# Benny44/QPALM

Measured on AMD Instinct MI355X. Metric: QP solves/sec (batched random n=1000,m=2000); `value` = solve only, batch resident in HBM -- with qpalm_setup in the clock as the reference's run_time has it: `value_setup_plus_solve`, higher is better.
Workload: dtype f64

## Files before the change

### qpalm_amd/csrc/qpalm_dense.h

```cpp
#ifndef QPALM_DENSE_H
#define QPALM_DENSE_H
#include <type_traits>

#ifdef QPALM_EMU
#define QP_FLAG_LOAD(p) (*(volatile int *)(p))
#define QP_FLAG_STORE(p, v) (*(volatile int *)(p) = (v))
#define QP_RELEASE_AGENT() do { } while (0)
#define QP_ACQUIRE_AGENT() do { } while (0)
#define QP_DRAIN_VMEM() do { } while (0)
#define QP_SLEEP() do { } while (0)
#define QP_WAVE_SYNC() emu_wave_sync()
#define QP_LDS_VBASE(p) (p)
#define QP_SCHED_BARRIER() do { } while (0)
#define QP_SETPRIO(p) do { } while (0)
#define QP_DRAIN_LDS() do { } while (0)
#else
#define QP_FLAG_LOAD(p) __hip_atomic_load((p), __ATOMIC_RELAXED, __HIP_MEMORY_SCOPE_AGENT)
#define QP_FLAG_STORE(p, v) __hip_atomic_store((p), (v), __ATOMIC_RELAXED, __HIP_MEMORY_SCOPE_AGENT)
#define QP_RELEASE_AGENT() __builtin_amdgcn_fence(__ATOMIC_RELEASE, "agent")
#define QP_ACQUIRE_AGENT() __builtin_amdgcn_fence(__ATOMIC_ACQUIRE, "agent")
#define QP_DRAIN_VMEM() asm volatile("s_waitcnt vmcnt(0)" ::: "memory")
#define QP_SLEEP() __builtin_amdgcn_s_sleep(2)
#define QP_SETPRIO(p) __builtin_amdgcn_s_setprio(p)
#define QP_DRAIN_LDS() asm volatile("s_waitcnt lgkmcnt(0)" ::: "memory")
// ... 771 lines not shown
  constexpr int NB = CO_SNB;
  const int tid = threadIdx.x, lane = tid & 63, wid = tid >> 6;
  const int jb = (n - J < NB) ? (n - J) : NB;
  __syncthreads();
  for (int e = tid; e < NB * NB; e += QP_T) {
    const int c = e / NB, r = e % NB;
    T.tile[r][c] = (r > c && r < jb) ? L[(size_t)(J + c) * ld + (J + r)] : 0.0;
  }
  __syncthreads();
  if (wid == 0) {
    double v = (lane < jb) ? x[J + lane] : 0.0;
#pragma unroll 8
    for (int c = 0; c < NB; c++) {
      const double yc = qp_readlane(v, c);
      v = QP_FMA(-T.tile[lane][c], yc, v);
    }
    T.part[lane] = v;
    if (wg == 0 && lane < jb) xo[J + lane] = v;
  }
  __syncthreads();
  for (int i = J + jb + wg * QP_T + tid; i < n; i += QP_T * nwg) {
    double acc = x[i];
#pragma unroll 1
    for (int c0 = 0; c0 < NB; c0 += 16) {
      double lv[16];
#pragma unroll
      for (int c = 0; c < 16; c++) lv[c] = QP_LDNT(3, &L[(size_t)(J + ((c0 + c < jb) ? c0 + c : jb - 1)) * ld + i]);
#pragma unroll
      for (int c = 0; c < 16; c++) if (c0 + c < jb) acc = QP_FMA(-lv[c], T.part[c0 + c], acc);
    }
    x[i] = acc;
  }
}
QPN void co_solve_backward(const double *L_, int n, int ld, double *x_, double *xo_, char *lds_, int J, int wg, int nwg) {
  const qp_gdouble *L = (const qp_gdouble *)L_;
  qp_gdouble *x = (qp_gdouble *)x_, *xo = (qp_gdouble *)xo_;
  CoSolveLds QP_LDS_AS &T = *QP_LDS_ARG(CoSolveLds, lds_);
  constexpr int NB = CO_SNB;
  const int tid = threadIdx.x, lane = tid & 63, wid = tid >> 6;
  const int jb = (n - J < NB) ? (n - J) : NB;
  __syncthreads();
  for (int e = tid; e < NB * NB; e += QP_T) {
    const int c = e / NB, r = e % NB;
    T.tile[r][c] = (r > c && r < jb) ? L[(size_t)(J + c) * ld + (J + r)] : 0.0;
  }
  __syncthreads();
  if (wid == 0) {
    double v = (lane < jb) ? x[J + lane] : 0.0;
#pragma unroll 8
    for (int r = NB - 1; r >= 0; r--) {
      const double xr = qp_readlane(v, r);
      v = QP_FMA(-T.tile[r][lane], xr, v);
    }
    T.part[lane] = (lane < jb) ? v : 0.0;
    if (wg == 0 && lane < jb) xo[J + lane] = v;
  }
  __syncthreads();
  const int grp = tid >> 4, gl = tid & 15, ngrp = QP_T / 16;
  double xb[4];
#pragma unroll
  for (int k = 0; k < 4; k++) xb[k] = T.part[4 * gl + k];
  for (int c0 = (wg * ngrp); c0 < J; c0 += ngrp * nwg) {
    const int c = c0 + grp;
    double s = 0.0;
    if (c < J) {
      const int r0 = J + 4 * gl;
      double lv[4];
#pragma unroll
      for (int k = 0; k < 4; k++) lv[k] = (r0 + k < n) ? QP_LDNT(3, &L[(size_t)c * ld + r0 + k]) : 0.0;
      s = QP_FMA(lv[1], xb[1], lv[0] * xb[0]);
      s = QP_FMA(lv[2], xb[2], s);
      s = QP_FMA(lv[3], xb[3], s);
    }
    for (int o = 8; o > 0; o >>= 1) s += __shfl_xor(s, o);
    if (c < J && gl == 0) x[c] = x[c] - s;
  }
}

#define QP_UNB 32
#ifndef QP_UNBS
#define QP_UNBS QP_UNB
#endif
#ifndef QP_UNBS32
#define QP_UNBS32 16
#endif
#ifndef QP_USQ
#define QP_USQ 1
#endif
#ifndef QP_TQD
#define QP_TQD 4
#endif
#define QP_CWG(U, buf, col) (U).cwg[buf][col]
template <int K> struct UpdownCfg {
  static constexpr int NB = (K > 16) ? QP_UNBS32 : QP_UNBS;
  static constexpr int G = (K + 15) / 16;
  static constexpr int KG = K / G;
};
template <int RPT, int K>
struct UpdownLds {
  static constexpr int NB = UpdownCfg<K>::NB;
  double Ld[2][NB][NB + 1];
  double Lsq[QP_USQ ? 2 : 1][QP_USQ ? NB : 1][NB];
  double Wd[2][NB][K + 1];
  double cwg[2][NB][K][2];
  double stash[RPT][K][64];
  double Wt[K];
  double dd[2][NB];
  double ys[2][NB];
  double stash_acc[RPT][64];
};

#ifdef QPALM_EMU
template <int N> QPD double qp_row_shr(double v) {
  const int lane = threadIdx.x & 63;
  const bool ok = (lane & 15) >= N;
  const double r = emu_exchange(v, ok ? lane - N : lane);
  return ok ? r : 0.0;
}
#else
template <int N> QPD double qp_row_shr(double v) {
  int lo = __double2loint(v), hi = __double2hiint(v);
  lo = __builtin_amdgcn_update_dpp(0, lo, 0x110 + N, 0xf, 0xf, true);
  hi = __builtin_amdgcn_update_dpp(0, hi, 0x110 + N, 0xf, 0xf, true);
  return __hiloint2double(hi, lo);
}
#endif
template <int KG> QPD double qp_rank_pivots_seq(const double p, const int ln, const double d0) {
  double run = d0 + p;
#pragma unroll
  for (int sq = 1; sq < KG; sq++) {
    const double up = qp_row_shr<1>(run);
    if ((ln & 15) == sq) run = up + p;
  }
  return run;
}
template <int KG> QPD int qp_rank_pivots(const double p, const int ln, const double d0, const int mode, double &dnew, double &dprev) {
  if (mode != QP_PIV_SEQ) {
    double incl = p;
    if (KG > 1) incl += qp_row_shr<1>(incl);
    if (KG > 2) incl += qp_row_shr<2>(incl);
    if (KG > 4) incl += qp_row_shr<4>(incl);
    if (KG > 8) incl += qp_row_shr<8>(incl);
    const double excl = qp_row_shr<1>(incl);
    dnew = d0 + incl; dprev = d0 + excl;
    if (mode == QP_PIV_TREE) return 0;
    const bool danger = !(__builtin_fabs(dnew) >= 0x1p-8 * __builtin_fabs(d0));
    if (__ballot(danger ? 1 : 0) == 0ull) return 0;
  }
  dnew = qp_rank_pivots_seq<KG>(p, ln, d0);
  const double sh = qp_row_shr<1>(dnew);
  dprev = ((ln & 15) == 0) ? d0 : sh;
  return (mode != QP_PIV_SEQ) ? 1 : 0;
}


#ifdef QPALM_EMU
template <int R> QPD double qp_row_bcast(double v) { const int lane = threadIdx.x & 63; return emu_exchange(v, (lane & ~15) | R); }
#else
template <int R> QPD double qp_row_bcast(double v) {
  return __builtin_amdgcn_update_dpp(0.0, v, 0x150 + R, 0xf, 0xf, true);
}
#endif
#ifdef QPALM_EMU
template <int K, int OFF, int R0, int R1, bool FIRST = true>
QPD void qp_apply_ranks_dpp(const double cw0, const double cw1, double (&wrow)[K], double &l) {
  const int lane = threadIdx.x & 63;
  emu_publish2(cw0, cw1);
  for (int r = R0; r < R1 && OFF + r < K; r++) {
    const double c0 = emu_peek((lane & ~15) | r, 0), c1 = emu_peek((lane & ~15) | r, 1);
    wrow[OFF + r] = QP_FMA(c0, l, wrow[OFF + r]);
    l = QP_FMA(c1, wrow[OFF + r], l);
  }
  emu_wave_sync();
}
#else
#ifndef QP_FMAC_DPP
#define QP_FMAC_DPP 1
#endif
#define QP_FD_STEP(i, n) "v_fmac_f64_dpp %" #i ", %9, %8 row_newbcast:%" #n " row_mask:0xf bank_mask:0xf bound_ctrl:1\n\t" \
                         "v_fmac_f64_dpp %8, %10, %" #i " row_newbcast:%" #n " row_mask:0xf bank_mask:0xf bound_ctrl:1\n\t"
#define QP_FD_EIGHT QP_FD_STEP(0, 11) QP_FD_STEP(1, 12) QP_FD_STEP(2, 13) QP_FD_STEP(3, 14) QP_FD_STEP(4, 15) QP_FD_STEP(5, 16) QP_FD_STEP(6, 17) QP_FD_STEP(7, 18)
template <int R0> QPD void qp_fmac_bcast8(double *w, double &l, const double cw0, const double cw1) {
  asm("s_nop 1\n\t" QP_FD_EIGHT
      : "+&v"(w[0]), "+&v"(w[1]), "+&v"(w[2]), "+&v"(w[3]), "+&v"(w[4]), "+&v"(w[5]), "+&v"(w[6]), "+&v"(w[7]), "+&v"(l)
      : "v"(cw0), "v"(cw1), "n"(R0), "n"(R0 + 1), "n"(R0 + 2), "n"(R0 + 3), "n"(R0 + 4), "n"(R0 + 5), "n"(R0 + 6), "n"(R0 + 7));
}
template <int K, int OFF, int R0, int R1, bool FIRST = true>
QPD void qp_apply_ranks_dpp(const double cw0, const double cw1, double (&wrow)[K], double &l) {
  if constexpr (QP_FMAC_DPP && R1 - R0 == 8 && OFF + R1 <= K) {
    qp_fmac_bcast8<R0>(&wrow[OFF + R0], l, cw0, cw1);
  } else if constexpr (R0 < R1 && OFF + R0 < K) {
    const double c0 = qp_row_bcast<R0>(cw0), c1 = qp_row_bcast<R0>(cw1);
    wrow[OFF + R0] = QP_FMA(c0, l, wrow[OFF + R0]);
    l = QP_FMA(c1, wrow[OFF + R0], l);
    qp_apply_ranks_dpp<K, OFF, R0 + 1, R1, false>(cw0, cw1, wrow, l);
  }
}
#endif
#ifndef QP_RECUR_DPP
#define QP_RECUR_DPP 1
#endif
#ifndef QP_AQD
#define QP_AQD 4
#endif
#ifndef QP_OWN_A
#define QP_OWN_A 1
#endif
#ifndef QP_SQ_WB
#define QP_SQ_WB 0
#endif
#ifndef QP_PANEL_A_DPP
#define QP_PANEL_A_DPP (K <= 16)
#endif
#ifndef QP_OWNER_DPP32
#define QP_OWNER_DPP32 1
#endif

template <int RPT, int K>
#ifndef QP_NI_UPDOWN
#define QP_NI_UPDOWN QPNI
#endif
QP_NI_UPDOWN void dense_updown(const int *Atp_, const int *Ati_, const double *Atss_, const int n_, const int ld_,
                               double *L_, double *Dg_, double *Wst_, const int *cols_, int n_up_,
                               const int *cols_dn_, int n_dn_, QpShared *S_, char *lds, int64_t *tdbg_, int pre_jmin_ = -1,
                               double *fs_ = nullptr, int rk0_ = 0, int rkn_ = 0x7fffffff) {
  const int n = QP_UNIFORM(n_), ld = QP_UNIFORM(ld_), n_up = QP_UNIFORM(n_up_), n_dn = QP_UNIFORM(n_dn_);
  const int rk0 = QP_UNIFORM(rk0_), rkn = QP_UNIFORM(rkn_);
  const int pre_jmin = QP_UNIFORM(pre_jmin_);
  const int pivmode = QP_UNIFORM(S_->seq_ranks);
  qp_gdouble *fs = (qp_gdouble *)fs_;
  const bool fuse_any = QP_UNIFORM((int)(fs_ != nullptr)) != 0;
  int64_t QP_LDS_AS *tdbg = (int64_t QP_LDS_AS *)tdbg_;
  const qp_gint *Atp = (const qp_gint *)Atp_, *Ati = (const qp_gint *)Ati_, *cols = (const qp_gint *)cols_, *cols_dn = (const qp_gint *)cols_dn_;
  const qp_gdouble *Atss = (const qp_gdouble *)Atss_;
  qp_gdouble *L = (qp_gdouble *)L_, *Dg = (qp_gdouble *)Dg_, *Wst = (qp_gdouble *)Wst_;
  QpShared &S = *S_;
  static_assert(K == 8 || K == 16 || K == 32, "rank groups of one DPP row (16 lanes), eight ranks at a time");
  static_assert(K <= QPG_KWST, "the staging area holds QPG_KWST dense update vectors");
  typedef UpdownLds<RPT, K> UpdownLdsT;
  UpdownLdsT QP_LDS_AS &U = *QP_LDS_ARG(UpdownLdsT, lds);
  static_assert(sizeof(UpdownLds<RPT, K>) <= ((RPT == 1) ? QP_LDS_BUDGET : QPG_LDS_DEFAULT), "update scratch must fit the dynamic LDS (the 256-thread instance only ever runs RPT = 1)");
  constexpr int NB = UpdownCfg<K>::NB, G = UpdownCfg<K>::G, KG = UpdownCfg<K>::KG;
  constexpr int PROWS = QP_T * RPT;
  constexpr bool MP = (K > 16);
  static_assert(PROWS % NB == 0, "passes start on block boundaries");
  const int lane = threadIdx.x & 63, wid = QP_UNIFORM(S.wave_rank[threadIdx.x >> 6]), tid = wid * 64 + lane;
  const int nr_all = n_up + n_dn;
  const int rk1 = (rkn < nr_all - rk0) ? (rk0 + rkn) : nr_all;
  qp_gdouble *dummy = Wst + (size_t)QPG_KWST * n;
  qp_gdouble *Tab = dummy + QPG_DUMMY + QPG_HSTASH;
  const int npass = MP ? (n + PROWS - 1) / PROWS : 1;
  for (int r0 = rk0; r0 < rk1; r0 += K) {
    const int kk = (rk1 - r0 < K) ? (rk1 - r0) : K;
    const bool fuse = fuse_any && (r0 + K >= nr_all);
    __syncthreads();
    long long tq0 = QP_CLOCK();
    int jmin = n;
    if (pre_jmin < 0) {
      for (int e = tid; e < kk * n; e += QP_T) Wst[e] = 0.0;
      __syncthreads();
      for (int r = wid; r < kk; r += QP_NW) {
        const int g = r0 + r;
        const int t = (g < n_up) ? cols[g] : cols_dn[g - n_up];
        for (int k = Atp[t] + lane; k < Atp[t + 1]; k += 64) {
          const int i = Ati[k];
          Wst[(size_t)r * n + i] = Atss[k];
          jmin = (i < jmin) ? i : jmin;
        }
      }
    } else jmin = (pre_jmin < n) ? pre_jmin : n - 1;
    if (fuse) jmin = 0;
    jmin = QP_UNIFORM(block_imin(S, jmin));
    double alpha[G], ialpha[G], sg[G];
    const int rl = QP_RECUR_DPP ? (lane & 15) : lane;
#pragma unroll
    for (int g = 0; g < G; g++) {
      alpha[g] = 1.0; ialpha[g] = 1.0;
      sg[g] = (16 * g + rl < kk) ? ((r0 + 16 * g + rl < n_up) ? 1.0 : -1.0) : 0.0;
    }
    const int J0 = (jmin / NB) * NB;
    if (tid == 0) {
      const long long tq1 = QP_CLOCK(); tdbg[0] += tq1 - tq0; tq0 = tq1;
      tdbg[QPG_CNT_SWEEPS] += 1;
      tdbg[QPG_CNT_SWEEP_ENTRIES] += (long long)(n - J0) * (n - J0 - 1) / 2 + (n - J0);
    }
    for (int pass = 0; pass < npass; pass++) {
    const int R0 = pass * PROWS;
    const int R1 = (!MP || n - R0 < PROWS) ? n : R0 + PROWS;
    const int Js = (J0 > R0) ? J0 : R0;
    if (Js >= R1) continue;
    const bool last_pass = (R1 >= n);
    const int rlim = last_pass ? ld : R1;
    if (MP && npass > 1) __syncthreads();
    double w[RPT][K];
#pragma unroll
    for (int rr = 0; rr < RPT; rr++) {
      const int i = R0 + tid * RPT + rr;
#pragma unroll
      for (int r = 0; r < K; r++) w[rr][r] = (i < R1 && r < kk) ? Wst[(size_t)r * n + i] : 0.0;
    }
    double acc[RPT];
#pragma unroll
    for (int rr = 0; rr < RPT; rr++) { const int i = R0 + tid * RPT + rr; acc[rr] = (fuse && i < R1) ? fs[i] : 0.0; }
    auto apply_table = [&](const int tb, const int Jc, const bool ok) QP_ALWAYS_INLINE {
      constexpr int QD = (K > 16) ? 2 * QP_TQD : QP_TQD;
      static_assert(NB % QD == 0, "queue depth divides the block");
      constexpr bool ODPP = QP_OWNER_DPP32 && (K > 16);
      const qp_pair QP_LDS_AS *tabO = (const qp_pair QP_LDS_AS *)QP_LDS_VBASE(&QP_CWG(U, tb, 0)[lane & 15][0]);
      const int i0 = R0 + tid * RPT;
      qp_gdouble *rowp = ok ? (L + (size_t)Jc * ld + i0) : (dummy + tid * RPT);
      const size_t cstride = ok ? (size_t)ld : 0;
      double q[QD][RPT];
#pragma unroll
      for (int cc = 0; cc < QD; cc++) qp_load_rows_nt<RPT>(rowp + (size_t)cc * cstride, q[cc]);
      auto group = [&](const int c0) QP_ALWAYS_INLINE {
#pragma unroll
        for (int u = 0; u < QD; u++) {
          int c1 = c0 + u;
          QP_OPAQUE(c1);
          double l[RPT];
          const int cpre = (c1 + QD < NB) ? c1 + QD : NB - 1;
#pragma unroll
          for (int rr = 0; rr < RPT; rr++) l[rr] = q[u][rr];
          if constexpr (ODPP) {
            qp_pair cf[G];
#pragma unroll
            for (int g = 0; g < G; g++) cf[g] = tabO[c1 * K + 16 * g];
#pragma unroll
            for (int rr = 0; rr < RPT; rr++) {
              qp_apply_ranks_dpp<K, 0, 0, 8, false>(cf[0].x, cf[0].y, w[rr], l[rr]);
              if (KG > 8 && kk > 8) qp_apply_ranks_dpp<K, 0, 8, 16, false>(cf[0].x, cf[0].y, w[rr], l[rr]);
              if constexpr (G > 1) {
                if (kk > 16) qp_apply_ranks_dpp<K, 16, 0, 8, false>(cf[G - 1].x, cf[G - 1].y, w[rr], l[rr]);
                if (kk > 24) qp_apply_ranks_dpp<K, 16, 8, 16, false>(cf[G - 1].x, cf[G - 1].y, w[rr], l[rr]);
              }
            }
          } else {
#pragma unroll
          for (int rb = 0; rb < K; rb += 4) {
            if (rb >= kk) break;
            double cf[4][2];
#pragma unroll
            for (int r = 0; r < 4; r++) {
              cf[r][0] = (rb + r < K) ? QP_CWG(U, tb, c1)[rb + r][0] : 0.0; cf[r][1] = (rb + r < K) ? QP_CWG(U, tb, c1)[rb + r][1] : 0.0;
            }
#pragma unroll
            for (int r = 0; r < 4; r++) {
              if (rb + r < K) {
#pragma unroll
                for (int rr = 0; rr < RPT; rr++) {
                  w[rr][rb + r] = QP_FMA(cf[r][0], l[rr], w[rr][rb + r]);
                  l[rr] = QP_FMA(cf[r][1], w[rr][rb + r], l[rr]);
                }
              }
            }
            QP_SCHED_BARRIER();
          }
          }
          qp_store_rows_nt<RPT>(rowp + (size_t)c1 * cstride, l);
          if (fuse) {
            const double yv = U.ys[tb][c1];
#pragma unroll
            for (int rr = 0; rr < RPT; rr++) acc[rr] = QP_FMA(-l[rr], yv, acc[rr]);
          }
          QP_SCHED_BARRIER();
          qp_load_rows_nt<RPT>(rowp + (size_t)cpre * cstride, q[u]);
          QP_SCHED_BARRIER();
        }
      };
      group(0);
#pragma unroll 1
      for (int c0 = QD; c0 < NB; c0 += QD) group(c0);
    };
    auto export_table = [&](const int tb, const int Jc, const int t0, const int nt) QP_ALWAYS_INLINE {
      const qp_pair QP_LDS_AS *src = (const qp_pair QP_LDS_AS *)&U.cwg[tb][0][0][0];
      for (int e = t0; e < NB * K; e += nt) {
        const qp_pair v = src[e];
        Tab[((size_t)Jc * K + e) * 2] = v.x; Tab[((size_t)Jc * K + e) * 2 + 1] = v.y;
      }
    };
    if constexpr (MP) if (R0 > J0) {
      const int nrb = (R0 - J0) / NB;
      const int i0 = R0 + tid * RPT;
      const bool ok = (i0 < rlim);
      constexpr int NE = (NB * K + QP_T - 1) / QP_T;
      qp_pair stg[NE];
      double ystg = 0.0;
      auto tab_load = [&](const int b) QP_ALWAYS_INLINE {
        const int Jc = J0 + b * NB;
#pragma unroll
        for (int q = 0; q < NE; q++) {
          const int e = tid + q * QP_T;
          if (e < NB * K) { stg[q].x = Tab[((size_t)Jc * K + e) * 2]; stg[q].y = Tab[((size_t)Jc * K + e) * 2 + 1]; }
        }
        if (fuse && tid < NB) ystg = fs[Jc + tid];
      };
      auto tab_store = [&](const int b) QP_ALWAYS_INLINE {
        qp_pair QP_LDS_AS *dst = (qp_pair QP_LDS_AS *)&U.cwg[b & 1][0][0][0];
#pragma unroll
        for (int q = 0; q < NE; q++) {
          const int e = tid + q * QP_T;
          if (e < NB * K) dst[e] = stg[q];
        }
        if (fuse && tid < NB) U.ys[b & 1][tid] = ystg;
      };
      tab_load(0);
      tab_store(0);
      __syncthreads();
      for (int b = 0; b < nrb; b++) {
        if (b + 1 < nrb) tab_load(b + 1);
        if (__ballot(ok ? 1 : 0) != 0ull) apply_table(b & 1, J0 + b * NB, ok);
        if (b + 1 < nrb) tab_store(b + 1);
        __syncthreads();
      }
    }
    const int nblk = (R1 - Js + NB - 1) / NB;
    {
      const int jb0 = (R1 - Js < NB) ? (R1 - Js) : NB;
#pragma unroll
      for (int rr = 0; rr < RPT; rr++) {
        const int i = R0 + tid * RPT + rr;
        if (i >= Js && i < Js + jb0) {
#pragma unroll
          for (int r = 0; r < K; r++) U.Wd[0][i - Js][r] = w[rr][r];
          U.Wd[0][i - Js][K] = acc[rr];
        }
      }
      for (int e = tid; e < jb0 * jb0; e += QP_T) {
        const int c1 = e / jb0, c = e % jb0;
        if (c > c1) U.Ld[0][c][c1] = L[(size_t)(Js + c1) * ld + (Js + c)];
      }
      if (tid < jb0) U.dd[0][tid] = Dg[Js + tid];
      if (wid == 0) {
#pragma unroll
        for (int rr = 0; rr < RPT; rr++)
#pragma unroll
          for (int r = 0; r < K; r++) U.stash[rr][r][lane] = w[rr][r];
#pragma unroll
        for (int rr = 0; rr < RPT; rr++) U.stash_acc[rr][lane] = acc[rr];
      }
    }
    if (tid == 0) { const long long tq1 = QP_CLOCK(); tdbg[0] += tq1 - tq0; tq0 = tq1; }
    __syncthreads();
    for (int s = 0; s < nblk; s++) {
      const int J = Js + s * NB, Jp = J - NB, Jn = J + NB;
      const int jb = (R1 - J < NB) ? (R1 - J) : NB;
      const int jbn = (R1 - Jn < NB) ? ((R1 - Jn > 0) ? (R1 - Jn) : 0) : NB;
      const int cur = s & 1, prv = cur ^ 1;
      long long tpe = QP_CLOCK();
      constexpr bool OWNA = QP_OWN_A && QP_USQ && !QP_SQ_WB;
      const int Ja = (OWNA && s > 0) ? J : Jn;
      const bool own_live0 = (R0 + 64 * RPT - 1 >= Ja);
      auto owner_block = [&]() QP_ALWAYS_INLINE {
        const long long tt0 = QP_CLOCK();
        bool any = false;
#pragma unroll
        for (int rr = 0; rr < RPT; rr++) { const int i = R0 + tid * RPT + rr; any = any || (i >= Ja && i < R1); }
        constexpr bool WAVES = MP && QP_OWNER_DPP32;
        if (s > 0 && (WAVES ? (__ballot(any ? 1 : 0) != 0ull) : any)) {
          const int i0 = R0 + tid * RPT;
          apply_table(prv, Jp, i0 >= Ja && i0 < rlim);
        }
#pragma unroll
        for (int rr = 0; rr < RPT; rr++) {
          const int i = R0 + tid * RPT + rr;
          if (i >= Jn && i < Jn + jbn) {
#pragma unroll
            for (int r = 0; r < K; r++) U.Wd[prv][i - Jn][r] = w[rr][r];
            U.Wd[prv][i - Jn][K] = acc[rr];
          }
        }
        if (wid == 0) {
#pragma unroll
          for (int rr = 0; rr < RPT; rr++)
#pragma unroll
            for (int r = 0; r < K; r++) U.stash[rr][r][lane] = w[rr][r];
#pragma unroll
          for (int rr = 0; rr < RPT; rr++) U.stash_acc[rr][lane] = acc[rr];
        }
        if (tid == QP_T - 64) tdbg[2] += QP_CLOCK() - tt0;
      };
      if (wid == 0) {
        const long long tp0 = QP_CLOCK();
        QP_SETPRIO(3);
        double wrow[K];
        double accp;
#pragma unroll
        for (int r = 0; r < K; r++) wrow[r] = (lane < jb) ? U.Wd[cur][lane][r] : 0.0;
        accp = (lane < jb) ? U.Wd[cur][lane][K] : 0.0;
        if (s > 0) {
          constexpr bool PSQ = QP_USQ;
          constexpr int QD = PSQ ? QP_AQD : 8;
          qp_gdouble *rowp = (lane < jb) ? (L + (size_t)Jp * ld + J + lane) : (dummy + lane);
          const size_t cstride = (lane < jb) ? (size_t)ld : 0;
          const int lrow = lane & (NB - 1);
          double q[QD];
#pragma unroll
          for (int cc = 0; cc < QD; cc++) q[cc] = PSQ ? U.Lsq[cur][cc][lrow] : rowp[(size_t)cc * cstride];
          const qp_pair QP_LDS_AS *tabA = (const qp_pair QP_LDS_AS *)QP_LDS_VBASE(&QP_CWG(U, prv, 0)[lane & 15][0]);
          qp_pair cfq[QP_PANEL_A_DPP ? QD : 1][G];
          if (QP_PANEL_A_DPP) {
#pragma unroll
            for (int cc = 0; cc < QD; cc++)
#pragma unroll
              for (int g = 0; g < G; g++) cfq[cc][g] = tabA[cc * K + 16 * g];
          }
          auto group = [&](const int c0) QP_ALWAYS_INLINE {
#pragma unroll
            for (int u = 0; u < QD; u++) {
              const int c1 = c0 + u;
              double l = q[u];
              const int cpre = (c1 + QD < NB) ? c1 + QD : NB - 1;
              if (QP_PANEL_A_DPP) {
                qp_apply_ranks_dpp<K, 0, 0, 8, false>(cfq[u][0].x, cfq[u][0].y, wrow, l);
                if (KG > 8 && kk > 8) qp_apply_ranks_dpp<K, 0, 8, 16, false>(cfq[u][0].x, cfq[u][0].y, wrow, l);
                if constexpr (G > 1) {
                  if (kk > 16) qp_apply_ranks_dpp<K, 16, 0, 8, false>(cfq[u][G - 1].x, cfq[u][G - 1].y, wrow, l);
                  if (kk > 24) qp_apply_ranks_dpp<K, 16, 8, 16, false>(cfq[u][G - 1].x, cfq[u][G - 1].y, wrow, l);
                }
              } else {
#pragma unroll
              for (int rb = 0; rb < K; rb += 8) {
                if (rb >= kk) break;
                double cw[8], cg[8];
#pragma unroll
                for (int r = 0; r < 8; r++) { cw[r] = (rb + r < K) ? QP_CWG(U, prv, c1)[rb + r][0] : 0.0; cg[r] = (rb + r < K) ? QP_CWG(U, prv, c1)[rb + r][1] : 0.0; }
#pragma unroll
                for (int r = 0; r < 8; r++) {
                  if (rb + r < K) {
                    wrow[rb + r] = QP_FMA(cw[r], l, wrow[rb + r]);
                    l = QP_FMA(cg[r], wrow[rb + r], l);
                  }
                }
                if (K > 16) QP_SCHED_BARRIER();
              }
              }
              if (PSQ && QP_SQ_WB) { if (lane < NB) U.Lsq[cur][c1][lrow] = l; }
              else if (!OWNA) rowp[(size_t)c1 * cstride] = l;
              if (fuse) accp = QP_FMA(-l, U.ys[prv][c1], accp);
              QP_SCHED_BARRIER();
              q[u] = PSQ ? U.Lsq[cur][cpre][lrow] : rowp[(size_t)cpre * cstride];
              if (QP_PANEL_A_DPP) {
#pragma unroll
                for (int g = 0; g < G; g++) cfq[u][g] = tabA[cpre * K + 16 * g];
              }
              QP_SCHED_BARRIER();
            }
          };
          group(0);
#pragma unroll 1
          for (int c0 = QD; c0 < NB; c0 += QD) group(c0);
        }
        if (QP_PANEL_TIMING == 1 && lane == 0) tdbg[8] += QP_CLOCK() - tp0;
        const long long tp1 = QP_CLOCK();
        double dreg = (lane < jb) ? U.dd[cur][lane] : 1.0;
        double lnext = (lane > 0 && lane < jb) ? U.Ld[cur][lane][0] : 0.0;
        double QP_LDS_AS *const wt = QP_LDS_VBASE(&U.Wt[0]);
#pragma unroll 1
        for (int c1 = 0; c1 < jb; c1++) {
          const int ln = QP_FRESH_LANE(lane);
          const double lcur = lnext;
          lnext = (ln > c1 + 1 && ln < jb) ? U.Ld[cur][ln][c1 + 1] : 0.0;
          long long tc0 = 0;
          if (QP_PANEL_TIMING == 2) { QP_DRAIN_LDS(); tc0 = QP_CLOCK(); }
          if (ln == c1) {
#pragma unroll
            for (int r = 0; r < K; r++) wt[r] = wrow[r];
          }
          QP_WAVE_SYNC();
          const int rk = QP_RECUR_DPP ? (ln & 15) : ln;
          double d0 = qp_readlane(dreg, c1);
          double nwv[G], ngam[G];
#pragma unroll
          for (int g = 0; g < G; g++) {
            const int kkg = (kk - 16 * g < KG) ? (kk - 16 * g) : KG;
            nwv[g] = 0.0; ngam[g] = 0.0;
            if (g > 0 && kkg <= 0) continue;
            const double wv = (rk < kkg) ? wt[(16 * g + rk) & (K - 1)] : 0.0;
            if (QP_PANEL_TIMING == 2 && g == 0) { QP_DRAIN_LDS(); const long long t = QP_CLOCK(); if (lane == 0) tdbg[8] += t - tc0; tc0 = t; }
            const double p = sg[g] * wv * wv * ialpha[g];
            double dnew, dprev;
            if (qp_rank_pivots<KG>(p, ln, d0, pivmode, dnew, dprev) && lane == 0) tdbg[QPG_CNT_SEQ_COLS] += 1;
            const double rdn = qp_rcp(dnew), rdp = qp_rcp(dprev);
            const double gam = -sg[g] * wv * ialpha[g] * rdn;
            if (ln < KG) { QP_CWG(U, cur, c1)[16 * g + ln][0] = -wv; QP_CWG(U, cur, c1)[16 * g + ln][1] = -gam; }
            alpha[g] = (wv == 0.0) ? alpha[g] : alpha[g] * dnew * rdp;
            ialpha[g] = (wv == 0.0) ? ialpha[g] : ialpha[g] * dprev * rdn;
            d0 = qp_readlane(dnew, kkg - 1);
            nwv[g] = -wv; ngam[g] = -gam;
          }
          if (QP_PANEL_TIMING == 2) { double gg = ngam[0]; QP_OPAQUE_V(gg); const long long t = QP_CLOCK(); if (lane == 0) tdbg[9] += t - tc0; tc0 = t; }
          if (ln == c1) dreg = d0;
          if (!QP_RECUR_DPP) QP_WAVE_SYNC();
          if (QP_RECUR_DPP) {
            double l = lcur;
            qp_apply_ranks_dpp<K, 0, 0, 8>(nwv[0], ngam[0], wrow, l);
            if (KG > 8 && kk > 8) qp_apply_ranks_dpp<K, 0, 8, 16, false>(nwv[0], ngam[0], wrow, l);
            if constexpr (G > 1) {
              if (kk > 16) qp_apply_ranks_dpp<K, 16, 0, 8>(nwv[1], ngam[1], wrow, l);
              if (kk > 24) qp_apply_ranks_dpp<K, 16, 8, 16, false>(nwv[1], ngam[1], wrow, l);
            }
            if (ln > c1 && ln < jb) U.Ld[cur][ln][c1] = l;
            if (QP_PANEL_TIMING == 2) { double ll = l; QP_OPAQUE_V(ll); const long long t = QP_CLOCK(); if (lane == 0) tdbg[11] += t - tc0; }
          } else {
            static_assert(QP_RECUR_DPP || G == 1, "the LDS form of the recurrence handles one rank group");
            double l = lcur;
            const qp_pair QP_LDS_AS *tab = (const qp_pair QP_LDS_AS *)&QP_CWG(U, cur, c1)[0][0];
            qp_pair cf[8];
#pragma unroll
            for (int r = 0; r < 8; r++) cf[r] = tab[r];
            if (QP_PANEL_TIMING == 2) { QP_DRAIN_LDS(); const long long t = QP_CLOCK(); if (lane == 0) tdbg[10] += t - tc0; tc0 = t; }
            if (K > 8 && kk > 8) {
#pragma unroll
              for (int r = 0; r < 8; r++) {
                wrow[r] = QP_FMA(cf[r].x, l, wrow[r]);
                l = QP_FMA(cf[r].y, wrow[r], l);
                cf[r] = tab[(8 + r < K) ? 8 + r : r];
                QP_SCHED_BARRIER();
              }
#pragma unroll
              for (int r = 0; r < 8; r++) {
                if (8 + r < K) {
                  wrow[8 + r] = QP_FMA(cf[r].x, l, wrow[8 + r]);
                  l = QP_FMA(cf[r].y, wrow[8 + r], l);
                }
              }
            } else {
#pragma unroll
              for (int r = 0; r < 8; r++) {
                wrow[r] = QP_FMA(cf[r].x, l, wrow[r]);
                l = QP_FMA(cf[r].y, wrow[r], l);
              }
            }
            if (ln > c1 && ln < jb) U.Ld[cur][ln][c1] = l;
            if (QP_PANEL_TIMING == 2) { double ll = l; QP_OPAQUE_V(ll); const long long t = QP_CLOCK(); if (lane == 0) tdbg[11] += t - tc0; }
          }
          QP_SCHED_BARRIER();
        }
        if (QP_PANEL_TIMING == 1 && lane == 0) tdbg[9] += QP_CLOCK() - tp1;
        const long long tp2 = QP_CLOCK();
        if (fuse) {
          double v = accp;
          double lc = (lane > 0 && lane < jb) ? U.Ld[cur][lane][0] : 0.0;
#pragma unroll 1
          for (int c = 0; c < jb; c++) {
            const int ln = QP_FRESH_LANE(lane);
            const double lcn = (ln > c + 1 && ln < jb) ? U.Ld[cur][ln][c + 1] : 0.0;
            const double yc = qp_readlane(v, c);
            v = QP_FMA(-lc, yc, v);
            lc = lcn;
          }
          if (lane < jb) { U.ys[cur][lane] = v; fs[J + lane] = v; }
        }
        if (lane < jb) Dg[J + lane] = dreg;
        if (!QP_USQ) {
#pragma unroll 1
          for (int c = 0; c < jb; c++)
            if (lane > c && lane < jb) L[(size_t)(J + c) * ld + (J + lane)] = U.Ld[cur][lane][c];
        }
#pragma unroll
        for (int rr = 0; rr < RPT; rr++)
#pragma unroll
          for (int r = 0; r < K; r++) w[rr][r] = own_live0 ? U.stash[rr][r][lane] : 0.0;
#pragma unroll
        for (int rr = 0; rr < RPT; rr++) acc[rr] = own_live0 ? U.stash_acc[rr][lane] : 0.0;
        QP_SETPRIO(0);
        if (lane == 0) { tdbg[1] += QP_CLOCK() - tp0; tdbg[QPG_CNT_SWEEP_COLS] += jb; }
        if (QP_PANEL_TIMING == 1 && lane == 0) tdbg[10] += QP_CLOCK() - tp2;
        tpe = QP_CLOCK();
      }
      if (wid != 0 || own_live0) owner_block();
      constexpr int NFREE = (QP_NW == 1) ? 0 : 1;
      if (wid >= NFREE) {
        const int t0 = tid - 64 * NFREE, nt = QP_T - 64 * NFREE;
        if (QP_USQ) {
          for (int e = t0; e < NB * NB; e += nt) {
            const int c1 = e / NB, c = e % NB;
            if (c > c1) {
              if (s > 0) L[(size_t)(Jp + c1) * ld + (Jp + c)] = U.Ld[prv][c][c1];
              if (c < jbn) U.Ld[prv][c][c1] = L[(size_t)(Jn + c1) * ld + (Jn + c)];
            }
            if (QP_SQ_WB && s >= 2) L[(size_t)(Jp - NB + c1) * ld + (Jp + c)] = U.Lsq[prv][c1][c];
            if (jbn > 0) U.Lsq[prv][c1][c] = (c < jbn) ? L[(size_t)(J + c1) * ld + (Jn + c)] : 0.0;
          }
        } else {
          for (int e = t0; e < jbn * jbn; e += nt) {
            const int c1 = e / jbn, c = e % jbn;
            if (c > c1) U.Ld[prv][c][c1] = L[(size_t)(Jn + c1) * ld + (Jn + c)];
          }
        }
        if (t0 < jbn) U.dd[prv][t0] = Dg[Jn + t0];
        if (MP && !last_pass && s > 0) export_table(prv, Jp, t0, nt);
      }
      __syncthreads();
      if (QP_PANEL_TIMING == 1 && tid == 0) tdbg[11] += QP_CLOCK() - tpe;
    }
    if (QP_USQ) {
      const int sl = nblk - 1, Jl = Js + sl * NB, jbl = R1 - Jl;
      for (int e = tid; e < NB * NB; e += QP_T) {
        const int c1 = e / NB, c = e % NB;
        if (c > c1 && c < jbl) L[(size_t)(Jl + c1) * ld + (Jl + c)] = U.Ld[sl & 1][c][c1];
        if (QP_SQ_WB && sl >= 1 && c < jbl) L[(size_t)(Jl - NB + c1) * ld + (Jl + c)] = U.Lsq[sl & 1][c1][c];
      }
    }
    if (MP && !last_pass) export_table((nblk - 1) & 1, Js + (nblk - 1) * NB, tid, QP_T);
    }
    if (tid == 0) { const long long tq1 = QP_CLOCK(); tdbg[7] += tq1 - tq0; tq0 = tq1; }
  }
  __syncthreads();
}


template <int K>
struct UpdownBigLds {
  double Ld[QP_UNB][QP_UNB + 1];
  double cwg[QP_UNB][K][2];
  double Wt[K];
  double dd[QP_UNB];
};
#ifndef QP_PANEL_DPP
#define QP_PANEL_DPP 1
#endif
template <int K>
QPD void updown_big_panel(UpdownBigLds<K> QP_LDS_AS &U, const int lane, const int jb, const int kk, const double sg,
                          double (&wrow)[K], double &dreg, double &alpha, double &ialpha, const int pivmode = QP_PIV_TREE) {
  static_assert(K == 16 || !QP_PANEL_DPP, "the DPP form needs one rank per lane of a 16-lane row");
  double lnext = (lane > 0 && lane < jb) ? U.Ld[lane][0] : 0.0;
#pragma unroll 1
  for (int c1 = 0; c1 < jb; c1++) {
    const int ln = QP_FRESH_LANE(lane);
    const double lcur = lnext;
    lnext = (ln > c1 + 1 && ln < jb) ? U.Ld[ln][c1 + 1] : 0.0;
    if (ln == c1) {
#pragma unroll
      for (int r = 0; r < K; r++) U.Wt[r] = wrow[r];
    }
    QP_WAVE_SYNC();
    const int rk = QP_PANEL_DPP ? (ln & (K - 1)) : ln;
    const double wv = (rk < kk) ? U.Wt[rk & (K - 1)] : 0.0;
    const double d0 = qp_readlane(dreg, c1);
    const double p = sg * wv * wv * ialpha;
    double dnew, dprev;
    qp_rank_pivots<K>(p, ln, d0, pivmode, dnew, dprev);
    const double rdn = qp_rcp(dnew), rdp = qp_rcp(dprev);
    const double gam = -sg * wv * ialpha * rdn;
    if (ln < K) { U.cwg[c1][ln][0] = -wv; U.cwg[c1][ln][1] = -gam; }
    alpha = (wv == 0.0) ? alpha : alpha * dnew * rdp;
    ialpha = (wv == 0.0) ? ialpha : ialpha * dprev * rdn;
    { const double dfin = qp_readlane(dnew, kk - 1); if (ln == c1) dreg = dfin; }
    if (QP_PANEL_DPP) {
      double l = lcur;
      qp_apply_ranks_dpp<K, 0, 0, 8>(-wv, -gam, wrow, l);
      if (K > 8 && kk > 8) qp_apply_ranks_dpp<K, 0, 8, 16>(-wv, -gam, wrow, l);
      if (ln > c1 && ln < jb) U.Ld[ln][c1] = l;
    } else {
      QP_WAVE_SYNC();
      double l = lcur;
#pragma unroll
      for (int r = 0; r < K; r++) {
        if (r >= kk) break;
        wrow[r] = QP_FMA(U.cwg[c1][r][0], l, wrow[r]);
        l = QP_FMA(U.cwg[c1][r][1], wrow[r], l);
      }
      if (ln > c1 && ln < jb) U.Ld[ln][c1] = l;
    }
    QP_SCHED_BARRIER();
  }
}

template <int K>
QPNI void dense_updown_big(const int *Atp_, const int *Ati_, const double *Atss_, const int n_, const int ld_,
                           double *L_, double *Dg_, double *Wst_, const int *cols_, int n_up_,
                           const int *cols_dn_, int n_dn_, QpShared *S_, char *lds, int64_t *tdbg_, int pre_jmin_ = -1) {
  const int n = QP_UNIFORM(n_), ld = QP_UNIFORM(ld_), n_up = QP_UNIFORM(n_up_), n_dn = QP_UNIFORM(n_dn_), pre_jmin = QP_UNIFORM(pre_jmin_);
  int64_t QP_LDS_AS *tdbg = (int64_t QP_LDS_AS *)tdbg_;
  const qp_gint *Atp = (const qp_gint *)Atp_, *Ati = (const qp_gint *)Ati_, *cols = (const qp_gint *)cols_, *cols_dn = (const qp_gint *)cols_dn_;
  const qp_gdouble *Atss = (const qp_gdouble *)Atss_;
  qp_gdouble *L = (qp_gdouble *)L_, *Dg = (qp_gdouble *)Dg_, *Wst = (qp_gdouble *)Wst_;
  QpShared &S = *S_;
  typedef UpdownBigLds<K> LdsT;
  LdsT QP_LDS_AS &U = *QP_LDS_ARG(LdsT, lds);
  const int NB = QP_UNB;
  const int tid = threadIdx.x, lane = tid & 63, wid = tid >> 6;
  const int nr = n_up + n_dn;
  for (int r0 = 0; r0 < nr; r0 += K) {
    const int kk = (nr - r0 < K) ? (nr - r0) : K;
    __syncthreads();
    long long tq0 = QP_CLOCK();
    int jmin = n;
    if (pre_jmin < 0) {
      for (int e = tid; e < kk * n; e += QP_T) Wst[e] = 0.0;
      __syncthreads();
      for (int r = wid; r < kk; r += QP_NW) {
        const int g = r0 + r;
        const int t = (g < n_up) ? cols[g] : cols_dn[g - n_up];
        for (int k = Atp[t] + lane; k < Atp[t + 1]; k += 64) {
          const int i = Ati[k];
          Wst[(size_t)r * n + i] = Atss[k];
          jmin = (i < jmin) ? i : jmin;
        }
      }
    } else jmin = (pre_jmin < n) ? pre_jmin : n - 1;
    jmin = QP_UNIFORM(block_imin(S, jmin));
    double alpha = 1.0, ialpha = 1.0;
    const int rl = QP_PANEL_DPP ? (lane & (K - 1)) : lane, grank = r0 + rl;
// ... 304 lines not shown
```

Before: 5346.

## Split 32-rank panel sweep into two pipelined 16-lane row groups

For rank groups of 32, the single-wave panel sweep now splits the ranks into two 16-rank halves handled by adjacent DPP rows. The second half trails the first by one column and receives the updated L value via permlane16_swap, so the two halves run as a skewed pipeline instead of one long serial chain of 32 rank updates per column. Pivot handling gains a per-row fallback so only the row that hits a dangerous pivot drops to the sequential path. This adds an extra pipeline step per loop, duplicated bookkeeping for alpha, pivots and the fused solve, and more register and code complexity.

```diff
diff --git a/qpalm_amd/csrc/qpalm_dense.h b/qpalm_amd/csrc/qpalm_dense.h
--- a/qpalm_amd/csrc/qpalm_dense.h
+++ b/qpalm_amd/csrc/qpalm_dense.h
@@ -947,6 +947,27 @@
   dprev = ((ln & 15) == 0) ? d0 : sh;
   return (mode != QP_PIV_SEQ) ? 1 : 0;
 }
+template <int KG> QPD int qp_rank_pivots_rows(const double p, const int ln, const double d0, const int mode, double &dnew, double &dprev) {
+  bool mine = true;
+  if (mode != QP_PIV_SEQ) {
+    double incl = p;
+    if (KG > 1) incl += qp_row_shr<1>(incl);
+    if (KG > 2) incl += qp_row_shr<2>(incl);
+    if (KG > 4) incl += qp_row_shr<4>(incl);
+    if (KG > 8) incl += qp_row_shr<8>(incl);
+    const double excl = qp_row_shr<1>(incl);
+    dnew = d0 + incl; dprev = d0 + excl;
+    if (mode == QP_PIV_TREE) return 0;
+    const bool danger = !(__builtin_fabs(dnew) >= 0x1p-8 * __builtin_fabs(d0));
+    const unsigned long long bal = __ballot(danger ? 1 : 0);
+    if (bal == 0ull) return 0;
+    mine = ((bal >> (ln & 48)) & 0xffffull) != 0ull;
+  }
+  const double run = qp_rank_pivots_seq<KG>(p, ln, d0);
+  const double sh = qp_row_shr<1>(run);
+  if (mine) { dnew = run; dprev = ((ln & 15) == 0) ? d0 : sh; }
+  return (mode != QP_PIV_SEQ && mine) ? 1 : 0;
+}
 
 
 #ifdef QPALM_EMU
@@ -968,6 +989,18 @@
   }
   emu_wave_sync();
 }
+template <int K, int OFF, int R0, int R1>
+QPD void qp_apply_ranks_dpp_en(const double cw0, const double cw1, double (&wrow)[K], double &l, const bool en) {
+  const int lane = threadIdx.x & 63;
+  emu_publish2(cw0, cw1);
+  for (int r = R0; en && r < R1 && OFF + r < K; r++) {
+    const double c0 = emu_peek((lane & ~15) | r, 0), c1 = emu_peek((lane & ~15) | r, 1);
+    wrow[OFF + r] = QP_FMA(c0, l, wrow[OFF + r]);
+    l = QP_FMA(c1, wrow[OFF + r], l);
+  }
+  emu_wave_sync();
+}
+QPD double qp_row_pair_down(double v) { const int lane = threadIdx.x & 63; return emu_exchange(v, lane & ~16); }
 #else
 #ifndef QP_FMAC_DPP
 #define QP_FMAC_DPP 1
@@ -991,6 +1024,26 @@
     qp_apply_ranks_dpp<K, OFF, R0 + 1, R1, false>(cw0, cw1, wrow, l);
   }
 }
+template <int R0> QPD void qp_fmac_bcast8_en(double *w, double &l, const double cw0, const double cw1) {
+  asm("s_nop 4\n\t" QP_FD_EIGHT
+      : "+&v"(w[0]), "+&v"(w[1]), "+&v"(w[2]), "+&v"(w[3]), "+&v"(w[4]), "+&v"(w[5]), "+&v"(w[6]), "+&v"(w[7]), "+&v"(l)
+      : "v"(cw0), "v"(cw1), "n"(R0), "n"(R0 + 1), "n"(R0 + 2), "n"(R0 + 3), "n"(R0 + 4), "n"(R0 + 5), "n"(R0 + 6), "n"(R0 + 7));
+}
+template <int K, int OFF, int R0, int R1>
+QPD void qp_apply_ranks_dpp_en(const double cw0, const double cw1, double (&wrow)[K], double &l, const bool en) {
+  static_assert(R1 - R0 == 8 && OFF + R1 <= K, "eight ranks at a time");
+  if constexpr (QP_FMAC_DPP) { if (en) qp_fmac_bcast8_en<R0>(&wrow[OFF + R0], l, cw0, cw1); }
+  else { if (en) qp_apply_ranks_dpp<K, OFF, R0, R1, false>(cw0, cw1, wrow, l); }
+}
+QPD double qp_row_pair_down(double v) {
+  typedef unsigned qp_u2 __attribute__((ext_vector_type(2)));
+  const qp_u2 a = __builtin_amdgcn_permlane16_swap((unsigned)__double2loint(v), (unsigned)__double2loint(v), false, false);
+  const qp_u2 b = __builtin_amdgcn_permlane16_swap((unsigned)__double2hiint(v), (unsigned)__double2hiint(v), false, false);
+  return __hiloint2double((int)b.x, (int)a.x);
+}
+#endif
+#ifndef QP_SPLIT32
+#define QP_SPLIT32 1
 #endif
 #ifndef QP_RECUR_DPP
 #define QP_RECUR_DPP 1
@@ -1038,6 +1091,7 @@
   constexpr int NB = UpdownCfg<K>::NB, G = UpdownCfg<K>::G, KG = UpdownCfg<K>::KG;
   constexpr int PROWS = QP_T * RPT;
   constexpr bool MP = (K > 16);
+  constexpr bool SPL = MP && QP_SPLIT32 && QP_RECUR_DPP && QP_USQ && QP_OWN_A && !QP_SQ_WB;
   static_assert(PROWS % NB == 0, "passes start on block boundaries");
   const int lane = threadIdx.x & 63, wid = QP_UNIFORM(S.wave_rank[threadIdx.x >> 6]), tid = wid * 64 + lane;
   const int nr_all = n_up + n_dn;
@@ -1278,6 +1332,97 @@
       if (wid == 0) {
         const long long tp0 = QP_CLOCK();
         QP_SETPRIO(3);
+        double dreg;
+        long long tp2;
+        if constexpr (SPL) {
+          const int rw = lane & 15, grp = (lane >> 4) & 1;
+          const int kkA = (kk < 16) ? kk : 16, kkB = kk - 16;
+          double wrow[16];
+#pragma unroll
+          for (int r = 0; r < 16; r++) wrow[r] = (rw < jb) ? U.Wd[cur][rw][16 * grp + r] : 0.0;
+          double accp = (rw < jb) ? U.Wd[cur][rw][K] : 0.0;
+          if (s > 0) {
+            const qp_pair QP_LDS_AS *tabS = (const qp_pair QP_LDS_AS *)QP_LDS_VBASE(&QP_CWG(U, prv, 0)[16 * grp + rw][0]);
+            double lq = U.Lsq[cur][0][rw], lB = 0.0;
+            qp_pair cq = tabS[0];
+#pragma unroll 1
+            for (int t = 0; t <= NB; t++) {
+              const int ln = QP_FRESH_LANE(lane);
+              const int g = (ln >> 4) & 1, tn = t + 1 - g;
+              const double lqn = U.Lsq[cur][(t + 1 < NB) ? t + 1 : NB - 1][ln & 15];
+              const qp_pair cqn = tabS[((tn < NB) ? tn : NB - 1) * K];
+              double l = g ? lB : lq;
+              qp_apply_ranks_dpp_en<16, 0, 0, 8>(cq.x, cq.y, wrow, l, g ? (t >= 1 && kk > 16) : (t < NB));
+              qp_apply_ranks_dpp_en<16, 0, 8, 16>(cq.x, cq.y, wrow, l, g ? (t >= 1 && kk > 24) : (t < NB && kk > 8));
+              if (fuse && g && t >= 1) accp = QP_FMA(-l, U.ys[prv][t - 1], accp);
+              lB = qp_row_pair_down(l);
+              lq = lqn; cq = cqn;
+              QP_SCHED_BARRIER();
+            }
+          }
+          if (QP_PANEL_TIMING == 1 && lane == 0) tdbg[8] += QP_CLOCK() - tp0;
+          const long long tp1 = QP_CLOCK();
+          dreg = (lane < jb) ? U.dd[cur][lane] : 1.0;
+          double lnext = (grp == 0 && rw > 0 && rw < jb) ? U.Ld[cur][rw][0] : 0.0;
+          double lB = 0.0, dAprev = 1.0, nseq = 0.0;
+          double al = grp ? alpha[1] : alpha[0], ial = grp ? ialpha[1] : ialpha[0];
+          const double sgl = grp ? sg[1] : sg[0];
+          double QP_LDS_AS *const wt = QP_LDS_VBASE(&U.Wt[0]);
+#pragma unroll 1
+          for (int t = 0; t <= jb; t++) {
+            const int ln = QP_FRESH_LANE(lane);
+            const int g = (ln >> 4) & 1, rk = ln & 15, cm = t - g;
+            const bool valid = g ? (t >= 1) : (t < jb);
+            const double lcur = g ? lB : lnext;
+            lnext = (g == 0 && rk > t + 1 && rk < jb) ? U.Ld[cur][rk][t + 1] : 0.0;
+            if (ln < 32 && rk == cm) {
+#pragma unroll
+              for (int r = 0; r < 16; r++) wt[16 * g + r] = wrow[r];
+            }
+            QP_WAVE_SYNC();
+            const double dc = qp_readlane(dreg, (t < jb) ? t : 0);
+            const double d0 = g ? dAprev : dc;
+            const double wv = (valid && rk < (g ? kkB : kkA)) ? wt[16 * g + rk] : 0.0;
+            const double p = sgl * wv * wv * ial;
+            double dnew, dprev;
+            const int rs = qp_rank_pivots_rows<16>(p, ln, d0, pivmode, dnew, dprev);
+            nseq += (rs && valid && (g ? kkB : kkA) > 0) ? 1.0 : 0.0;
+            const double rdn = qp_rcp(dnew), rdp = qp_rcp(dprev);
+            const double gam = -sgl * wv * ial * rdn;
+            if (ln < 32 && valid) { QP_CWG(U, cur, cm)[16 * g + rk][0] = -wv; QP_CWG(U, cur, cm)[16 * g + rk][1] = -gam; }
+            al = (wv == 0.0) ? al : al * dnew * rdp;
+            ial = (wv == 0.0) ? ial : ial * dprev * rdn;
+            const double dA = qp_readlane(dnew, kkA - 1);
+            const double dB = (kkB > 0) ? qp_readlane(dnew, 16 + kkB - 1) : dAprev;
+            if (t >= 1 && ln == t - 1) dreg = dB;
+            dAprev = dA;
+            double l = lcur;
+            qp_apply_ranks_dpp_en<16, 0, 0, 8>(-wv, -gam, wrow, l, valid && (g == 0 || kk > 16));
+            qp_apply_ranks_dpp_en<16, 0, 8, 16>(-wv, -gam, wrow, l, valid && (g ? kk > 24 : kk > 8));
+            if (ln < 32 && valid && g == 1 && rk > cm && rk < jb) U.Ld[cur][rk][cm] = l;
+            lB = qp_row_pair_down(l);
+            QP_SCHED_BARRIER();
+          }
+          if (grp) { alpha[1] = al; ialpha[1] = ial; } else { alpha[0] = al; ialpha[0] = ial; }
+          const double ns = qp_readlane(nseq, 0) + qp_readlane(nseq, 16);
+          if (lane == 0 && ns != 0.0) tdbg[QPG_CNT_SEQ_COLS] += (long long)ns;
+          if (QP_PANEL_TIMING == 1 && lane == 0) tdbg[9] += QP_CLOCK() - tp1;
+          tp2 = QP_CLOCK();
+          if (fuse) {
+            double v = accp;
+            double lc = (grp == 1 && rw > 0 && rw < jb) ? U.Ld[cur][rw][0] : 0.0;
+#pragma unroll 1
+            for (int c = 0; c < jb; c++) {
+              const int ln = QP_FRESH_LANE(lane);
+              const int rk = ln & 15;
+              const double lcn = (((ln >> 4) & 1) == 1 && rk > c + 1 && rk < jb) ? U.Ld[cur][rk][c + 1] : 0.0;
+              const double yc = qp_readlane(v, 16 + c);
+              v = QP_FMA(-lc, yc, v);
+              lc = lcn;
+            }
+            if (grp == 1 && lane < 32 && rw < jb) { U.ys[cur][rw] = v; fs[J + rw] = v; }
+          }
+        } else {
         double wrow[K];
         double accp;
 #pragma unroll
@@ -1348,7 +1493,7 @@
         }
         if (QP_PANEL_TIMING == 1 && lane == 0) tdbg[8] += QP_CLOCK() - tp0;
         const long long tp1 = QP_CLOCK();
-        double dreg = (lane < jb) ? U.dd[cur][lane] : 1.0;
+        dreg = (lane < jb) ? U.dd[cur][lane] : 1.0;
         double lnext = (lane > 0 && lane < jb) ? U.Ld[cur][lane][0] : 0.0;
         double QP_LDS_AS *const wt = QP_LDS_VBASE(&U.Wt[0]);
 #pragma unroll 1
@@ -1433,7 +1578,7 @@
           QP_SCHED_BARRIER();
         }
         if (QP_PANEL_TIMING == 1 && lane == 0) tdbg[9] += QP_CLOCK() - tp1;
-        const long long tp2 = QP_CLOCK();
+        tp2 = QP_CLOCK();
         if (fuse) {
           double v = accp;
           double lc = (lane > 0 && lane < jb) ? U.Ld[cur][lane][0] : 0.0;
@@ -1446,6 +1591,7 @@
             lc = lcn;
           }
           if (lane < jb) { U.ys[cur][lane] = v; fs[J + lane] = v; }
+        }
         }
         if (lane < jb) Dg[J + lane] = dreg;
         if (!QP_USQ) {
```

After: 5345 (median of 2 runs). No clear change (-0.0%).
